# ArisKonidaris/OMLDM

Hardware: AMD Instinct MI355X
Metric: training examples/sec (whole node) + p50 predict latency, linear SVM 1/2/4/8 GPU (higher is better)
Workload: dtype fp32

## Files before the change

### csrc/kernels/linear_scan3.hip

```cpp
#include "common.h"
#include "hash_dev.h"
#include "seq_common.h"

namespace omldm {

typedef float f32x4 __attribute__((ext_vector_type(4)));

namespace s3 {
constexpr int CH = 64;
#ifndef OMLDM_S3_NH
#define OMLDM_S3_NH 11
#endif
constexpr int NH = OMLDM_S3_NH;
constexpr int NT = 64 * (NH + 1);
constexpr int WPE = (NH + 1 + 3) / 4;
constexpr int NHA = NH;
constexpr int GS = CH + 4;
constexpr int MAXF = 32;
constexpr int NF = (MAXF + NHA - 1) / NHA;
constexpr int KNMAX = 32;
constexpr int NJ = (KNMAX + NHA - 1) / NHA;
constexpr int MAT = CH * CH;
constexpr int RMAX = 8192;
constexpr int WS = 8;
constexpr int DS = KNMAX;
constexpr uint32_t F_TG = 1u;
constexpr uint32_t F_INIT = 2u;
constexpr uint32_t F_SCAT = 4u;
constexpr uint32_t F_SIGN = 8u;
constexpr uint32_t F_PRES = 16u;
constexpr uint32_t F_TAB = F_TG | F_INIT | F_SCAT;
constexpr int LID_SHIFT = 10;
}

template <int KN>
__host__ __device__ constexpr int s3_prep_floats() {
  return 2 * s3::MAT + s3::CH + KN * s3::CH + 3 * s3::CH;
}
template <int KN>
__host__ __device__ constexpr int s3_prep_y() {
  return 2 * s3::MAT + s3::CH + KN * s3::CH;
}
template <int KN>
__host__ __device__ constexpr int s3_prep_sg() {
  return s3_prep_y<KN>() + s3::CH;
}
template <int KN>
__host__ __device__ constexpr int s3_prep_hh() {
  return s3_prep_y<KN>() + 2 * s3::CH;
}
__device__ __forceinline__ float s3_shrink(int shr, float r, float tbase, int i, float y) {
  if (shr == 0 || y != y) return 1.f;
  if (shr == 2) {
    const float T = tbase + (float)i;
    return (T - 1.f) / T;
  }
  return r;
}

__device__ __forceinline__ void spoke_rows(int s, int R, int B, int& t0, int& t1) {
  const long long a = (long long)s * R;
  t0 = a > B ? B : (int)a;
  t1 = (a + R) > B ? B : (int)(a + R);
}

__global__ __launch_bounds__(256) void s3_slots_kernel(const void* __restrict__ src, int B,
                                                       int dc, int dn, uint32_t span, int hashed,
                                                       int cbase, int* __restrict__ slotsT) {
  __shared__ int tile[256][s3::MAXF + 1];
  const int r0 = blockIdx.x * 256, tid = threadIdx.x;
  const int nr = min(256, B - r0);
  for (int i = tid; i < nr * dc; i += 256) {
    const int r = i / dc, f = i - r * dc;
    int slot;
    if (hashed == 2) {
      const uint32_t v = reinterpret_cast<const uint16_t*>(src)[(size_t)r0 * dc + i];
      slot = v == 0xFFFFu ? -1
                          : (int)(((uint32_t)cbase + (uint32_t)f * span + (v & 0x7FFFu)) |
                                  ((v & 0x8000u) << 16));
    } else {
      const uint32_t v = reinterpret_cast<const uint32_t*>(src)[(size_t)r0 * dc + i];
      slot = hashed ? (int)v : hash_token_dev(v, f, dn, span);
    }
    tile[r][f] = slot;
  }
  __syncthreads();
  if (tid < nr)
    for (int f = 0; f < dc; ++f) slotsT[(size_t)f * B + r0 + tid] = tile[tid][f];
}

namespace s3 {
constexpr int FT = 1024;
constexpr int HCAP = 12288;
constexpr int RPT = RMAX / FT;
}

__global__ __launch_bounds__(s3::FT) void s3_flags_kernel(const int* __restrict__ slotsT, int B,
                                                          int R, uint32_t* __restrict__ meta,
                                                          int* __restrict__ lidcount, int enc,
                                                          int* __restrict__ l2s, long long gs) {
  __shared__ int hkey[s3::HCAP];
  __shared__ uint32_t hfirst[s3::HCAP];
  __shared__ uint32_t hlast[s3::HCAP];
  __shared__ int s_cnt, s_base;
// ... 621 lines not shown
  const int i = bid - base;
  s3_combine_spoke(slotsT, dc, B, R, cb, sm, i % cb.S_act, i / cb.S_act, (nblk - base) / cb.S_act);
}

__device__ void s3_dense_body(const float* __restrict__ ws, const float* __restrict__ wsd,
                              const float* __restrict__ sig, int S_act, int dn, int dim, int bias,
                              float inv_p, float* __restrict__ dacc, double* __restrict__ cum);

__device__ __forceinline__ void s3_scan_arrive(const S3Comb& cb, const float* __restrict__ ws,
                                               const float* __restrict__ wsd, int dn, int dim,
                                               const SeqParams& p, S3Smem& sm) {
  if (cb.arrive == nullptr) return;
  int& s_last = sm.last;
  asm volatile("s_waitcnt vmcnt(0)" ::: "memory");
  __syncthreads();
  if (threadIdx.x == 0) {
    __builtin_amdgcn_fence(__ATOMIC_RELEASE, "agent");
    asm volatile("s_waitcnt vmcnt(0)" ::: "memory");
    s3_gu64* a = (s3_gu64*)cb.arrive;
    unsigned long long old = __hip_atomic_load(a, __ATOMIC_RELAXED, __HIP_MEMORY_SCOPE_AGENT);
    unsigned long long nw;
    do {
      nw = (uint32_t)(old >> 32) == cb.epoch ? old + 1
                                             : (((unsigned long long)cb.epoch << 32) | 1ull);
    } while (!__hip_atomic_compare_exchange_weak(a, &old, nw, __ATOMIC_RELAXED,
                                                 __ATOMIC_RELAXED, __HIP_MEMORY_SCOPE_AGENT));
    s_last = (int)(uint32_t)nw == cb.S_act;
    if (s_last) {
      __builtin_amdgcn_fence(__ATOMIC_ACQUIRE, "agent");
      asm volatile("s_waitcnt vmcnt(0)" ::: "memory");
    }
  }
  __syncthreads();
  if (s_last)
    s3_dense_body(ws, wsd, cb.sig, cb.S_act, dn, dim, p.bias, p.inv_p, cb.dacc, cb.cum);
}

template <bool RARE>
__device__ __forceinline__ void s3_inscan_flush(const S3Comb& cb, const float* tab,
                                                float* ag, int cap,
                                                const float* __restrict__ w, int s) {
  __syncthreads();
  const int n = cb.lidcount[s];
  const float sc = cb.inv_p * (cb.sig ? cb.sig[s] : 1.f);
  const int* l2 = cb.l2s + (size_t)s * cb.gs;
  constexpr int FB = 8;
  for (int i0 = threadIdx.x; i0 < n; i0 += FB * s3::NT) {
    int slot[FB];
    float d[FB];
#pragma unroll
    for (int u = 0; u < FB; ++u) {
      const int i = i0 + u * s3::NT;
      slot[u] = l2[i < n ? i : 0];
    }
#pragma unroll
    for (int u = 0; u < FB; ++u) {
      const int i = i0 + u * s3::NT;
      d[u] = i < min(n, cap) ? tab[i] : 0.f;
    }
    if (n > cap) {
#pragma unroll
      for (int u = 0; u < FB; ++u) {
        const int i = i0 + u * s3::NT;
        if (i >= cap && i < n)
          d[u] = __hip_atomic_load(&ag[i - cap], __ATOMIC_RELAXED, __HIP_MEMORY_SCOPE_AGENT);
      }
    }
    if constexpr (!RARE) {
#pragma unroll
      for (int u = 0; u < FB; ++u) {
        const int i = i0 + u * s3::NT;
        const int sl = i < n ? slot[u] : 0;
        d[u] -= i < n ? (cb.wbf ? s3_w16(w, sl) : w[sl]) : 0.f;
      }
    }
#pragma unroll
    for (int u = 0; u < FB; ++u) {
      const int i = i0 + u * s3::NT;
      if (i < n && d[u] != 0.f) atomicAdd(&cb.dacc[slot[u]], sc * d[u]);
    }
  }
}

template <int RULE, int KN, bool RARE>
__device__ __forceinline__ void s3_scan_body(
    int bid, int nblk, S3Smem& sm, float* tab,
    const int* __restrict__ slotsT, const uint32_t* __restrict__ meta, int dc, int dn,
    const void* __restrict__ yv, int B, int R, const float* __restrict__ prep, int nchs,
    const float* __restrict__ w, int dim, float* __restrict__ aglob, int cap, long long gstride,
    const S3Comb& cb, float* __restrict__ ws, float* __restrict__ wsd, const SeqParams& p,
    unsigned long long* __restrict__ rgran) {
  constexpr int PF = s3_prep_floats<KN>();
  if (bid >= cb.S_act) {
    if (RARE && bid < 2 * cb.S_act) {
      s3_rare(slotsT, dc, B, R, w, cb, rgran, sm, bid - cb.S_act);
      if (cb.inscan == 2) s3_fold_pres(meta, dc, B, R, cb, bid - cb.S_act);
      return;
    }
    s3_combine(slotsT, dc, B, R, cb, sm, (RARE ? 2 : 1) * cb.S_act, bid, nblk);
    return;
  }
  const int tid = threadIdx.x;
  const int wave = __builtin_amdgcn_readfirstlane(tid >> 6), lane = tid & 63;
  const int s = bid;
  int t0, t1;
  spoke_rows(s, R, B, t0, t1);
  if (t0 >= t1) {
    if (tid < s3::WS) ws[(size_t)s * s3::WS + tid] = 0.f;
    if (tid < s3::DS) wsd[(size_t)s * s3::DS + tid] = 0.f;
    s3_scan_arrive(cb, ws, wsd, dn, dim, p, sm);
    return;
  }
  const int nch = (t1 - t0 + s3::CH - 1) / s3::CH;
  const float* P0 = prep + (size_t)s * nchs * PF;
  auto chunk_prep = [&](int k) { return P0 + (size_t)k * PF; };
  float* ag = aglob + (size_t)s * gstride;

  unsigned long long* stamps = g_s3_stamps;
  unsigned long long st_acc[12] = {};
  unsigned long long st_t = stamps ? clock64() : 0;
  auto stamp = [&](int k) {
    if (stamps) {
      const unsigned long long now = clock64();
      st_acc[k] += now - st_t;
      st_t = now;
    }
  };

  if (wave == 0) {
    __builtin_amdgcn_s_setprio(3);
    float loss = 0.f, nex = 0.f, mist = 0.f, sqe = 0.f;
    float f1 = 0.f;
    float ynx = chunk_prep(0)[s3_prep_y<KN>() + lane];
    float anx = chunk_prep(0)[2 * s3::MAT + lane];
    const bool shr = p.shr != 0;
    float snx = shr ? chunk_prep(0)[s3_prep_sg<KN>() + lane] : 1.f;
    float hnx = shr ? chunk_prep(0)[s3_prep_hh<KN>() + lane] : 1.f;
    for (int k = -1; k <= nch; ++k) {
      if (k >= 0 && k < nch) {
        const int b = k & 1;
        const int row = t0 + k * s3::CH + lane;
        const bool valid = row < t1 && ynx == ynx;
        const float y = valid ? ynx : 0.f;
        const float a = valid ? anx : 0.f;
        const float sg = valid ? snx : 1.f, hh = valid ? hnx : 1.f;
        if (k + 1 < nch) {
          ynx = chunk_prep(k + 1)[s3_prep_y<KN>() + lane];
          anx = chunk_prep(k + 1)[2 * s3::MAT + lane];
          if (shr) {
            snx = chunk_prep(k + 1)[s3_prep_sg<KN>() + lane];
            hnx = chunk_prep(k + 1)[s3_prep_hh<KN>() + lane];
          }
        }
        float m0 = 0.f;
#pragma unroll
        for (int q = 0; q < s3::NHA; ++q) m0 += sm.part[b][q][lane];
        S3Cand<RULE> cf;
        float u, bc = 0.f;
        const float inv = -a;
        if constexpr (RULE == kSeqHinge) {
          bc = y * inv * hh;
          cf.lo = y < 0.f ? -p.cclip * hh : 0.f;
          cf.hi = y < 0.f ? 0.f : (y > 0.f ? p.cclip * hh : 0.f);
          u = fmaf(a * (sg * hh), m0, bc) + f1;
        } else if constexpr (RULE == kSeqEps) {
          bc = (y - p.eps) * inv * hh;
          cf.d = 2.f * p.eps * inv * hh;
          cf.lo = valid ? -p.cclip * hh : 0.f;
          cf.hi = valid ? p.cclip * hh : 0.f;
          u = fmaf(a * (sg * hh), m0, bc) + f1;
        } else if constexpr (RULE == kSeqPegasos) {
          const float T = p.tbase + (float)(row - t0);
          cf.lo = valid ? 1.f / sg : 0.f;
          cf.hi = valid ? y * hh / (p.lam * T) : 0.f;
          u = fmaf(a, m0, 0.f) + f1;
        } else {
          cf.lo = y * sg;
          cf.hi = p.lr * y * hh;
          u = m0 + f1;
        }
        const float* grow = &sm.G[b][lane][0];
        const float* xrow = &sm.X1[b ^ 1][lane][0];
        float gg[s3::CH], xx[s3::CH];
#pragma unroll
        for (int t4 = 0; t4 < s3::CH; t4 += 4) {
          const float4 g4 = *reinterpret_cast<const float4*>(grow + t4);
          const float4 x4 = *reinterpret_cast<const float4*>(xrow + t4);
          gg[t4] = g4.x, gg[t4 + 1] = g4.y, gg[t4 + 2] = g4.z, gg[t4 + 3] = g4.w;
          xx[t4] = x4.x, xx[t4 + 1] = x4.y, xx[t4 + 2] = x4.z, xx[t4 + 3] = x4.w;
        }
        stamp(8);
        float n1 = 0.f;
        auto chain = [&](auto step) {
#pragma unroll
          for (int t = 0; t < s3::CH; ++t) {
            const float ct = readlane_f(step(u), t);
            u = fmaf(ct, gg[t], u);
            n1 = fmaf(ct, xx[t], n1);
            asm volatile("" : "+v"(u), "+v"(n1));
          }
        };
        if constexpr (RULE == kSeqLogistic) {
          if (!shr) {
            const float lo2 = y * 1.44269504088896341f;
            chain([&](float v) {
              return __builtin_amdgcn_rcpf(1.f + __builtin_amdgcn_exp2f(lo2 * v));
            });
          } else {
            chain([&](float v) { return cf(v, p, y); });
          }
        } else {
          chain([&](float v) { return cf(v, p, y); });
        }
        stamp(9);
        const float c = cf(u, p, y);
        sm.cb[b][lane] = c;
        if (row < t1 && cb.inscan != 1)
          __hip_atomic_store((s3_gu64*)(cb.gran + row),
                             ((unsigned long long)cb.epoch << 32) | __float_as_uint(c),
                             __ATOMIC_RELAXED, __HIP_MEMORY_SCOPE_AGENT);
        if (valid) {
          float m;
          if constexpr (RULE == kSeqLogistic) m = sg * u;
          else if constexpr (RULE == kSeqPegasos) m = sg * y * u;
          else m = inv > 0.f ? (bc - u) * __builtin_amdgcn_rcpf(inv * hh) : 0.f;
          seq_stats<RULE>(m, y, p, loss, mist, sqe);
          nex += 1.f;
        }
        f1 = n1;
      }
      stamp(0);
      __syncthreads();
      stamp(1);
    }
    if (stamps && lane == 0)
      for (int q = 0; q < 12; ++q)
        if (q < 2 || q >= 8) atomicAdd(&stamps[(size_t)s * 16 + q], st_acc[q]);
    loss = wave_sum(loss);
    nex = wave_sum(nex);
    mist = wave_sum(mist);
    sqe = wave_sum(sqe);
    if (lane == 0) {
      float* wr = ws + (size_t)s * s3::WS;
      wr[0] = loss;
      wr[1] = nex;
      wr[2] = mist;
      wr[3] = sqe;
      wr[4] = 1.f;
      wr[5] = 0.f;
      wr[6] = 0.f;
      wr[7] = 0.f;
    }
    if (cb.inscan) s3_inscan_flush<RARE>(cb, tab, ag, cap, w, s);
    s3_scan_arrive(cb, ws, wsd, dn, dim, p, sm);
    return;
  }

  const int q = wave - 1, r = lane;
  const int swave = g_s3_stamp_wave;
  const int kd = dn + (p.bias ? 1 : 0);
  const int hl = q * 64 + lane;
  const bool inscan = cb.inscan != 0, inscan1 = cb.inscan == 1;
  const uint32_t tmask = inscan ? s3::F_TAB : s3::F_SCAT;
  const float isc = inscan1 ? cb.inv_p * (cb.sig ? cb.sig[s] : 1.f) : 0.f;
  float wn[s3::NJ], w0[s3::NJ];
#pragma unroll
  for (int i = 0; i < s3::NJ; ++i) {
    const int j = q + s3::NHA * i;
    const int jw = j < dn ? j : dim - 1;
    const float wj = cb.wbf ? s3_w16(w, jw) : w[jw];
    w0[i] = (j < KN && (j < dn || (p.bias && j == dn))) ? wj : 0.f;
    wn[i] = w0[i];
  }
  constexpr int NV4 = (2 * s3::MAT / 4 + 64 * s3::NHA - 1) / (64 * s3::NHA);
  struct Set {
    int cs[s3::NF];
    uint32_t cm[s3::NF];
    float g[s3::NF];
    f32x4 v[NV4];
    float xs[s3::NJ], xc[s3::NJ];
    unsigned long long rg;
  };
  uint32_t p1[s3::NF], p2[s3::NF];
  const unsigned long long want = (unsigned long long)cb.epoch;
  bool dead = false;
  auto load_rare = [&](int ch) -> unsigned long long {
    const int row = t0 + ch * s3::CH + r;
    const bool ok = RARE && q == 0 && ch >= 0 && ch < nch && row < t1;
    return ok ? __hip_atomic_load((s3_gu64*)(rgran + row), __ATOMIC_RELAXED,
                                  __HIP_MEMORY_SCOPE_AGENT)
              : (want << 32);
  };
  auto load_words = [&](int ch, Set& S) {
    if constexpr (RARE) {
      S.rg = load_rare(ch);
#pragma unroll
      for (int i = 0; i < s3::NF; ++i) {
        const int f = q + s3::NHA * i;
        const int row = t0 + ch * s3::CH + r;
        const bool ok = ch >= 0 && ch < nch && f < dc && row < t1;
        const uint32_t mm = meta[ok ? (size_t)f * B + row : 0];
        S.cm[i] = ok ? mm : 0u;
        S.cs[i] = ok && (mm & (s3::F_TG | s3::F_INIT)) ? 0 : -1;
      }
      return;
    }
#pragma unroll
    for (int i = 0; i < s3::NF; ++i) {
      const int f = q + s3::NHA * i;
      const int row = t0 + ch * s3::CH + r;
      const bool ok = ch >= 0 && ch < nch && f < dc && row < t1;
      const size_t at = ok ? (size_t)f * B + row : 0;
      const int sl = slotsT[at];
      const uint32_t mm = meta[at];
      S.cs[i] = ok ? sl : -1;
      S.cm[i] = ok ? mm : 0u;
    }
  };
  auto issue_gathers = [&](Set& S) {
    if constexpr (RARE) return;
    if (cb.wbf) {
#pragma unroll
      for (int i = 0; i < s3::NF; ++i) {
        const bool glob = !RARE && S.cs[i] != -1 && !(S.cm[i] & s3::F_TG);
        S.g[i] = s3_w16(w, glob ? (S.cs[i] & 0x7fffffff) : 0);
      }
      return;
    }
#pragma unroll
    for (int i = 0; i < s3::NF; ++i) {
      const bool glob = !RARE && S.cs[i] != -1 && !(S.cm[i] & s3::F_TG);
      S.g[i] = w[glob ? (S.cs[i] & 0x7fffffff) : 0];
    }
  };
  auto issue_staging = [&](int ch, Set& S) {
#pragma unroll
    for (int u = 0; u < NV4; ++u) {
      const int i = min(hl + 64 * s3::NHA * u, 2 * s3::MAT / 4 - 1);
      const int mtx = i >> 10, e = i & 1023;
      const int kc = max(0, min(ch + mtx, nch - 1));
      S.v[u] = reinterpret_cast<const f32x4*>(chunk_prep(kc) + mtx * s3::MAT)[e];
    }
  };
  constexpr int NJK = (KN + s3::NHA - 1) / s3::NHA;
  auto load_dense = [&](int ch, float* xd) {
#pragma unroll
    for (int i = 0; i < NJK; ++i) {
      const int j = q + s3::NHA * i;
      const bool ok = j < KN && ch >= 0 && ch < nch;
      const int jc = j < KN ? j : 0, cc = max(0, min(ch, nch - 1));
      const float v = chunk_prep(cc)[2 * s3::MAT + s3::CH + jc * s3::CH + r];
      xd[i] = ok ? v : 0.f;
    }
  };
  auto body = [&](auto spill_tag, int k, Set& CUR, Set& NXT) {
    constexpr bool SPILL = decltype(spill_tag)::value;
    const int cn = k + 1, ks = k - 1;
    if (wave == swave) stamp(7);
    load_words(cn + 1, NXT);
    issue_staging(cn + 1, NXT);
    load_dense(ks + 1, NXT.xs);
    load_dense(cn + 1, NXT.xc);
    if (wave == swave) stamp(3);
    if (ks >= 0) {
      const float cv = sm.cb[ks & 1][r];
#pragma unroll
      for (int i = 0; i < s3::NF; ++i) {
        const uint32_t m = p2[i];
        const bool sc = (m & tmask) != 0u && cv != 0.f;
        const bool dr = inscan1 && (m & s3::F_PRES) != 0u && cv != 0.f;
        if (__builtin_amdgcn_ballot_w64(sc || dr) == 0ull) continue;
        const int lid = (int)(m >> s3::LID_SHIFT);
        const float val = (m & s3::F_SIGN) ? -cv : cv;
        if (dr) atomicAdd(&cb.dacc[lid], val * isc);
        if (sc) {
          if constexpr (SPILL) {
            if (lid < cap) atomicAdd(&tab[lid], val);
            else atomicAdd(&ag[lid - cap], val);
          } else {
            atomicAdd(&tab[lid], val);
          }
        }
      }
#pragma unroll
      for (int i = 0; i < NJK; ++i) {
        const int j = q + s3::NHA * i;
        if (j < kd) wn[i] += wave_sum(cv * CUR.xs[i]);
      }
    }
    if (wave == swave) stamp(6);
    if (cn < nch) {
      float base = 0.f;
#pragma unroll
      for (int i = 0; i < NJK; ++i) base = fmaf(CUR.xc[i], wn[i], base);
      if constexpr (RARE) {
        if (q == 0) {
          for (unsigned spins = 0;
               __builtin_amdgcn_ballot_w64((CUR.rg >> 32) != want) != 0ull;) {
            if (dead || ++spins > s3::SPIN_MAX) {
              if (!dead && r == 0) atomicExch(&g_s3_comb_err, 2);
              dead = true;
              break;
            }
            __builtin_amdgcn_s_sleep(1);
            CUR.rg = load_rare(cn);
          }
          base += (CUR.rg >> 32) == want ? __uint_as_float((uint32_t)CUR.rg) : 0.f;
        }
      }
      if constexpr (!SPILL) {
        float tv[s3::NF];
#pragma unroll
        for (int i = 0; i < s3::NF; ++i) {
          const uint32_t m = CUR.cm[i];
          const bool tg = CUR.cs[i] != -1 && (m & s3::F_TG);
          tv[i] = 0.f;
          if (tg) tv[i] = tab[(int)(m >> s3::LID_SHIFT)];
        }
#pragma unroll
        for (int i = 0; i < s3::NF; ++i) {
          const uint32_t m = CUR.cm[i];
          const bool here = CUR.cs[i] != -1;
          const bool tg = here && (m & s3::F_TG), init = here && !tg && (m & s3::F_INIT);
          const float val = tg ? tv[i] : (RARE ? 0.f : CUR.g[i]);
          if (init) tab[(int)(m >> s3::LID_SHIFT)] = val;
          if (here && (!RARE || tg)) base += (m & s3::F_SIGN) ? -val : val;
        }
      }
#pragma unroll
      for (int i = 0; SPILL && i < s3::NF; ++i) {
        const uint32_t m = CUR.cm[i];
        const bool here = CUR.cs[i] != -1;
        const int lid = (int)(m >> s3::LID_SHIFT);
        const bool tg = here && (m & s3::F_TG), init = here && !tg && (m & s3::F_INIT);
        float val = RARE ? 0.f : CUR.g[i];
        if (!SPILL || __builtin_amdgcn_ballot_w64((tg || init) && lid >= cap) == 0ull) {
          if (tg) val = tab[lid];
          if (init) tab[lid] = val;
        } else if constexpr (SPILL) {
          if (tg) val = lid < cap ? tab[lid] : __hip_atomic_load(&ag[lid - cap], __ATOMIC_RELAXED,
                                                                 __HIP_MEMORY_SCOPE_WORKGROUP);
          if (init) {
            if (lid < cap) tab[lid] = val;
            else __hip_atomic_store(&ag[lid - cap], val, __ATOMIC_RELAXED,
                                    __HIP_MEMORY_SCOPE_WORKGROUP);
          }
          asm volatile("s_waitcnt vmcnt(0)" ::: "memory");
        }
        if (here && (!RARE || tg)) base += (m & s3::F_SIGN) ? -val : val;
      }
      sm.part[cn & 1][q][r] = base;
    }
    if (wave == swave) stamp(4);
#pragma unroll
    for (int u = 0; u < NV4; ++u) {
      const int i = hl + 64 * s3::NHA * u;
      const int mtx = i >> 10, e = i & 1023;
      if (i < 2 * s3::MAT / 4 && cn + mtx < nch) {
        const int row = e >> 4, col = (e & 15) * 4;
        float* dst = mtx == 0 ? &sm.G[cn & 1][row][col] : &sm.X1[(cn + 1) & 1][row][col];
        *reinterpret_cast<f32x4*>(dst) = CUR.v[u];
      }
    }
    issue_gathers(NXT);
#pragma unroll
    for (int i = 0; i < s3::NF; ++i) {
      p2[i] = p1[i];
      p1[i] = CUR.cm[i];
    }
    if (wave == swave) stamp(5);
    __syncthreads();
  };

  Set A, Bs;
#pragma unroll
  for (int i = 0; i < s3::NF; ++i) p1[i] = p2[i] = 0u;
  load_words(0, A);
  issue_staging(0, A);
  load_dense(-2, A.xs);
  load_dense(0, A.xc);
  issue_gathers(A);
  if (cb.lidcount[s] <= cap) {
    for (int k = -1; k <= nch; k += 2) {
      body(S3Tag<false>{}, k, A, Bs);
      if (k + 1 <= nch) body(S3Tag<false>{}, k + 1, Bs, A);
    }
  } else {
    for (int k = -1; k <= nch; k += 2) {
      body(S3Tag<true>{}, k, A, Bs);
      if (k + 1 <= nch) body(S3Tag<true>{}, k + 1, Bs, A);
    }
  }
  if (stamps && lane == 0 && wave == swave)
    for (int k = 2; k < 8; ++k) atomicAdd(&stamps[(size_t)s * 16 + k], st_acc[k]);
#pragma unroll
  for (int i = 0; i < s3::NJ; ++i) {
    const int j = q + s3::NHA * i;
    if (lane == 0 && j < KN) wsd[(size_t)s * s3::DS + j] = wn[i] - w0[i];
  }
  if (q == 0 && lane >= KN && lane < s3::DS) wsd[(size_t)s * s3::DS + lane] = 0.f;
  if (cb.inscan) s3_inscan_flush<RARE>(cb, tab, ag, cap, w, s);
  s3_scan_arrive(cb, ws, wsd, dn, dim, p, sm);
}

constexpr int kS3MaxPipes = 16;
struct S3Pipe {
  const float* w;
  float* aglob;
  float* ws;
  float* wsd;
  unsigned long long* rgran;
  S3Comb cb;
  SeqParams p;
};
struct S3Pipes {
  int M;
  int ncomb;
  const unsigned long long* wflag;
  unsigned long long wepoch;
  S3Pipe pipe[kS3MaxPipes];
};

__global__ void s3_signal_kernel(unsigned long long* flag, unsigned long long epoch) {
  if (threadIdx.x == 0)
    __hip_atomic_store(flag, epoch, __ATOMIC_RELEASE, __HIP_MEMORY_SCOPE_AGENT);
}

__device__ __forceinline__ void s3_wait_prep(const unsigned long long* flag,
                                             unsigned long long epoch) {
  if (flag == nullptr) return;
  if (threadIdx.x == 0) {
    for (unsigned spins = 0;
         __hip_atomic_load(flag, __ATOMIC_RELAXED, __HIP_MEMORY_SCOPE_AGENT) < epoch;) {
      if (++spins > s3::SPIN_MAX) {
        atomicExch(&g_s3_comb_err, 3);
        break;
      }
      __builtin_amdgcn_s_sleep(2);
    }
    __builtin_amdgcn_fence(__ATOMIC_ACQUIRE, "agent");
  }
  __syncthreads();
}

template <int RULE, int KN, bool RARE>
__global__ __launch_bounds__(s3::NT, s3::WPE) __attribute__((amdgpu_waves_per_eu(s3::WPE, s3::WPE))) void s3_scan_kernel(
    const int* __restrict__ slotsT, const uint32_t* __restrict__ meta, int dc, int dn,
    const void* __restrict__ yv, int B, int R, const float* __restrict__ prep, int nchs,
    int dim, int cap, long long gstride, int S_act, S3Pipes pp) {
  __shared__ S3Smem sm;
  extern __shared__ float tab[];
  const int nblk = s3_nper(S_act, RARE, pp.ncomb);
  const int pi = (int)blockIdx.x / nblk, local = (int)blockIdx.x % nblk;
  s3_wait_prep(pp.wflag, pp.wepoch);
  int bid;
  if (RARE && local < S_act) bid = S_act + local;
  else if (RARE && local < 2 * S_act) bid = local - S_act;
  else bid = local;
  const S3Pipe& P = pp.pipe[pi];
  s3_scan_body<RULE, KN, RARE>(bid, nblk, sm, tab, slotsT, meta, dc, dn, yv, B, R, prep, nchs,
                               P.w, dim, P.aglob, cap, gstride, P.cb, P.ws, P.wsd, P.p, P.rgran);
}

__device__ void s3_dense_body(const float* __restrict__ ws,
                              const float* __restrict__ wsd, const float* __restrict__ sig,
                              int S_act, int dn, int dim, int bias, float inv_p,
                              float* __restrict__ dacc,
                              double* __restrict__ cum) {
  const int tid = threadIdx.x;
  const bool bad = __hip_atomic_load(&g_s3_comb_err, __ATOMIC_RELAXED, __HIP_MEMORY_SCOPE_AGENT) != 0;
  for (int i = tid; i < dn; i += 256) {
    float v = 0.f;
    for (int s = 0; s < S_act; ++s) v += wsd[(size_t)s * s3::DS + i] * (sig ? sig[s] : 1.f);
    dacc[i] = v * inv_p;
  }
  if (tid == 0) {
    float v = 0.f, a = 0.f;
    if (bias)
      for (int s = 0; s < S_act; ++s) v += wsd[(size_t)s * s3::DS + dn] * (sig ? sig[s] : 1.f);
    for (int s = 0; s < S_act; ++s) a += sig ? sig[s] : 1.f;
    dacc[dim - 1] = v * inv_p;
    dacc[dim] = a * inv_p;
    dacc[dim + 1] = bad ? -1e30f : (float)S_act * inv_p;
  }
  if (cum && !bad && tid < 6 && tid != 4) {
    double t = 0.0;
    for (int s = 0; s < S_act; ++s) t += (double)ws[(size_t)s * s3::WS + tid];
    cum[tid] += t;
  }
}

namespace s3 {
constexpr int SB = 4096;
constexpr int SH = 4096;
constexpr int SPROBE = 8;
}

__global__ __launch_bounds__(256) void s3_tail_kernel(const float* __restrict__ ws,
                                                      const float* __restrict__ wsd,
                                                      const float* __restrict__ sig, int S_act,
                                                      int dn, int dim, int bias, float inv_p,
                                                      float* __restrict__ dacc,
                                                      double* __restrict__ cum) {
  s3_dense_body(ws, wsd, sig, S_act, dn, dim, bias, inv_p, dacc, cum);
}

__global__ __launch_bounds__(256) void s3_scatter_kernel(const int* __restrict__ slotsT,
                                                         const unsigned long long* __restrict__ gran, int B,
                                                         int n_rows, float inv_p,
                                                         float* __restrict__ dacc, int dc,
                                                         const float* __restrict__ ws,
                                                         const float* __restrict__ wsd, int S_act,
                                                         int dn, int dim, int bias,
                                                         double* __restrict__ cum, int R,
                                                         const float* __restrict__ sig) {
  if ((int)blockIdx.y == dc) {
    if (blockIdx.x == 0) s3_dense_body(ws, wsd, sig, S_act, dn, dim, bias, inv_p, dacc, cum);
    return;
  }
  __shared__ int hk[s3::SH];
  __shared__ float hv[s3::SH];
  const int f = blockIdx.y, tid = threadIdx.x;
  const int r0 = blockIdx.x * s3::SB, r1 = min(n_rows, r0 + s3::SB);
  for (int i = tid; i < s3::SH; i += 256) {
    hk[i] = -1;
    hv[i] = 0.f;
  }
  __syncthreads();
  const int* col = slotsT + (size_t)f * B;
  for (int row = r0 + tid; row < r1; row += 256) {
    const int v = col[row];
    if (v == -1) continue;
    const float c = __uint_as_float((uint32_t)gran[row]);
    if (c == 0.f) continue;
    const int key = v & 0x7fffffff;
    const float sc = sig ? inv_p * sig[row / R] : inv_p;
    const float val = v < 0 ? -c * sc : c * sc;
    uint32_t at = ((uint32_t)key * 0x9E3779B1u) >> (32 - 12);
    bool done = false;
    for (int probe = 0; probe < s3::SPROBE; ++probe) {
      const int prev = atomicCAS(&hk[at], -1, key);
      if (prev == -1 || prev == key) {
        atomicAdd(&hv[at], val);
// ... 484 lines not shown
  }
#pragma unroll
  for (int i = 0; i < s3::NJ; ++i) {
    const int j = q + s3::NHA * i;
    if (lane == 0 && j < s3::DS)
#pragma unroll
      for (int c = 0; c < K; ++c)
        A.wsd[((size_t)s * K + c) * s3::DS + j] =
            (i < NJK0 && j < KN) ? wn[c][i < NJK0 ? i : 0] - w0_at(i, c) : 0.f;
  }
  if (hdbg && lane == 0) {
    atomicAdd(&hdbg[s * 8 + 3], h_sc);
    atomicAdd(&hdbg[s * 8 + 4], h_mg);
    atomicAdd(&hdbg[s * 8 + 5], h_st);
    atomicAdd(&hdbg[s * 8 + 6], h_wt);
    if (q == 0) atomicAdd(&hdbg[s * 8 + 7], (unsigned long long)(lidcount[s] > capid));
  }
}

__global__ __launch_bounds__(256) void s3mc_scatter_kernel(
    const int* __restrict__ slotsT, const float* __restrict__ tau, const int* __restrict__ rr,
    const void* __restrict__ yv, int y8, int nclass, int B, int n_rows, float* __restrict__ dacc,
    int dim, int dc, int dn, int bias, int K, int KN, const float* __restrict__ ws,
    const float* __restrict__ wsd, int S_act, float* __restrict__ stats) {
  if ((int)blockIdx.y == dc) {
    if (blockIdx.x != 0) return;
    const int tid = threadIdx.x;
    for (int i = tid; i < K * KN; i += 256) {
      const int c = i / KN, j = i - c * KN;
      if (j >= dn + (bias ? 1 : 0) || c >= nclass) continue;
      float v = 0.f;
      for (int s = 0; s < S_act; ++s) v += wsd[((size_t)s * K + c) * s3::DS + j];
      const int key = j < dn ? j : dim - 1;
      dacc[(size_t)c * dim + key] += v;
    }
    if (tid < 3) {
      float t = 0.f;
      for (int s = 0; s < S_act; ++s) t += ws[(size_t)s * s3::WS + tid];
      stats[tid] += t;
    }
    if (tid == 3) stats[3] += (float)S_act;
    return;
  }
  __shared__ int hk[s3::SH];
  __shared__ float hv[s3::SH];
  const int f = blockIdx.y, tid = threadIdx.x;
  const int r0 = blockIdx.x * s3::SB, r1 = min(n_rows, r0 + s3::SB);
  for (int i = tid; i < s3::SH; i += 256) {
    hk[i] = -1;
    hv[i] = 0.f;
  }
  __syncthreads();
  const int* col = slotsT + (size_t)f * B;
  auto add = [&](int key, float val) {
    uint32_t at = ((uint32_t)key * 0x9E3779B1u) >> (32 - 12);
    for (int probe = 0; probe < s3::SPROBE; ++probe) {
      const int prev = atomicCAS(&hk[at], -1, key);
      if (prev == -1 || prev == key) {
        atomicAdd(&hv[at], val);
        return;
      }
      at = (at + 1) & (s3::SH - 1);
    }
    atomicAdd(&dacc[key], val);
  };
  for (int row = r0 + tid; row < r1; row += 256) {
    const int v = col[row];
    const float t = tau[row];
    if (v == -1 || t == 0.f) continue;
    const int slot = v & 0x7fffffff;
    const float val = v < 0 ? -t : t;
    const float yf = load_y(yv, row, y8);
    const int yc = (yf == yf && yf >= 0.f && yf < (float)nclass) ? (int)yf : -1;
    if (yc >= 0) add(yc * dim + slot, val);
    if (rr[row] >= 0) add(rr[row] * dim + slot, -val);
  }
  __syncthreads();
  for (int i = tid; i < s3::SH; i += 256) {
    const int key = hk[i];
    if (key != -1) atomicAdd(&dacc[key], hv[i]);
  }
}

template <int RULE, int KN, bool RARE>
static int s3_launch_scan_t(const int* slotsT, const uint32_t* meta, int dc, int dn, const void* y,
                            int B, int R, int S_act, const float* prep, int nchs, int dim, int cap,
                            long long gstride, const S3Pipes& pp, hipStream_t st) {
  static bool attr_set = false;
  if (!attr_set) {
    hipFuncSetAttribute(reinterpret_cast<const void*>(&s3_scan_kernel<RULE, KN, RARE>),
                        hipFuncAttributeMaxDynamicSharedMemorySize,
                        160 * 1024 - (int)sizeof(S3Smem));
    attr_set = true;
  }
  const int nblk = pp.M * s3_nper(S_act, RARE, pp.ncomb);
  hipLaunchKernelGGL((s3_scan_kernel<RULE, KN, RARE>), dim3(nblk), dim3(s3::NT),
                     (size_t)(cap + 64) * sizeof(float), st, slotsT, meta, dc, dn, y, B, R, prep,
                     nchs, dim, cap, gstride, S_act, pp);
  return (int)hipGetLastError();
}

template <int KN>
static int s3_launch_scan(int rule, bool rare, const int* slotsT, const uint32_t* meta, int dc,
                          int dn, const void* y, int B, int R, int S_act, const float* prep,
                          int nchs, int dim, int cap, long long gstride, const S3Pipes& pp,
                          hipStream_t st) {
#define OMLDM_S3L(RL, RA) \
  return s3_launch_scan_t<RL, KN, RA>(slotsT, meta, dc, dn, y, B, R, S_act, prep, nchs, dim, cap, \
                                      gstride, pp, st)
  if (rare) {
    if (rule == kSeqHinge) OMLDM_S3L(kSeqHinge, true);
    if (rule == kSeqEps) OMLDM_S3L(kSeqEps, true);
    if (rule == kSeqPegasos) OMLDM_S3L(kSeqPegasos, true);
    OMLDM_S3L(kSeqLogistic, true);
  }
  if (rule == kSeqHinge) OMLDM_S3L(kSeqHinge, false);
  if (rule == kSeqEps) OMLDM_S3L(kSeqEps, false);
  if (rule == kSeqPegasos) OMLDM_S3L(kSeqPegasos, false);
  OMLDM_S3L(kSeqLogistic, false);
#undef OMLDM_S3L
}

}

using namespace omldm;

namespace {
int s3_sact(int B, int R, int S) {
  const long long sact = ((long long)B + R - 1) / R;
  return sact < S ? (int)sact : S;
}
int s3_kn(int dn, int bias) { return dn + (bias ? 1 : 0) <= 16 ? 16 : 32; }
constexpr size_t kFlagsLds = (size_t)s3::HCAP * 12;
}

static int g_s3_cap_override = -1;

static int g_s3_mode = 4;
static int g_s3_inscan = 1;
OMLDM_API void omldm_scan3_set_inscan(int v) { g_s3_inscan = v; }
OMLDM_API void omldm_scan3_set_mode(int m) { g_s3_mode = m == 3 ? 3 : 4; }
OMLDM_API int omldm_scan3_get_mode() { return g_s3_mode; }

OMLDM_API int omldm_scan3_lds_cap() {
  const int hw = (int)((160 * 1024 - sizeof(S3Smem)) / sizeof(float)) - 64;
  return g_s3_cap_override >= 0 && g_s3_cap_override < hw ? g_s3_cap_override : hw;
}

OMLDM_API void omldm_scan3_set_cap(int cap) { g_s3_cap_override = cap; }

static int g_s3_gram_valu = 0;
OMLDM_API void omldm_scan3_set_gram_valu(int v) { g_s3_gram_valu = v; }

static int g_s3_comb = 1;
OMLDM_API void omldm_scan3_set_comb(int v) { g_s3_comb = v < 0 ? 0 : (v > 3 ? 3 : v); }
OMLDM_API int omldm_scan3_get_comb() { return g_s3_comb; }

OMLDM_API int omldm_scan3_comb_err() {
  int v = 0, z = 0;
  if (hipMemcpyFromSymbol(&v, HIP_SYMBOL(g_s3_comb_err), sizeof(v)) != hipSuccess) return -1;
  if (v) hipMemcpyToSymbol(HIP_SYMBOL(g_s3_comb_err), &z, sizeof(z));
  return v;
}

__global__ void s3_err_drain_kernel(int* out) {
  if (threadIdx.x == 0) {
    const int v = atomicExch(&g_s3_comb_err, 0);
    out[0] = v > out[0] ? v : out[0];
  }
}

OMLDM_API int omldm_scan3_comb_err_drain(int* out, void* stream) {
  hipLaunchKernelGGL(s3_err_drain_kernel, dim3(1), dim3(64), 0, (hipStream_t)stream, out);
  return (int)hipGetLastError();
}

OMLDM_API int omldm_scan3_fits(int dn, int dc, int R, int bias) {
  return dc > 0 && dc <= s3::MAXF && dn >= 0 && dn + (bias ? 1 : 0) <= s3::KNMAX && R > 0 &&
         R <= s3::RMAX;
}

OMLDM_API long long omldm_scan3_ws_words(int which, int B, int R, int S, int dn, int dc,
// ... 304 lines not shown
```

### omldm_amd/cli.py

```python
from __future__ import annotations

import json
import sys

from omldm_amd.utils.config import JobConfig, argparser


def main(argv=None) -> int:
    argv = list(sys.argv[1:] if argv is None else argv)
    if "-h" in argv or "--help" in argv:
        argparser().print_help()
        return 0
    cfg = JobConfig.from_args(argv)
    from omldm_amd.engine.job import Job
    from omldm_amd.parallel.comm import init_distributed

    comm, device = init_distributed(cfg.device)
    job = Job(cfg, comm, device).run()
    if comm.rank == 0:
        print(json.dumps({"job": cfg.jobName, "ticks": job.ticks, "counters": job.counters,
                          "terminated": job.terminated}), flush=True)
    return 0


if __name__ == "__main__":
    sys.exit(main())
```

### omldm_amd/parallel/comm.py

```python
from __future__ import annotations

import os
from dataclasses import dataclass, field

import torch
import torch.distributed as dist


_BYTE_WIRE = (torch.int16, torch.uint16, torch.bool) if hasattr(torch, "uint16") else \
    (torch.int16, torch.bool)


@dataclass
class CommStats:
    collectives: int = 0
    bytes: int = 0
    small_collectives: int = 0
    per_tag: dict = field(default_factory=dict)
    trace: list | None = None

    def add(self, tag: str, nbytes: int, small: bool = False, kind: str = "all_reduce"):
        if self.trace is not None:
            self.trace.append((kind, tag, int(nbytes)))
        self.collectives += 1
# ... 153 lines not shown
    def broadcast_(self, t: torch.Tensor, src: int = 0, tag: str = "bcast"):
        if self.world > 1:
            self.stats.add(tag, t.numel() * t.element_size(), kind="broadcast")
            dist.broadcast(t, src=src, group=self.group)

    def broadcast_object(self, obj, src: int = 0):
        if self.world == 1:
            return obj
        box = [obj if self.rank == src else None]
        dist.broadcast_object_list(box, src=src, group=self.group)
        return box[0]

    def all_gather_object(self, obj) -> list:
        if self.world == 1:
            return [obj]
        out = [None] * self.world
        dist.all_gather_object(out, obj, group=self.group)
        return out

    def gather_tensor(self, t: torch.Tensor, dst: int = 0) -> list[torch.Tensor] | None:
        if self.world == 1:
            return [t]
        n = torch.tensor([t.shape[0]], dtype=torch.int64)
        ns_t = [torch.zeros_like(n) for _ in range(self.world)] if self.rank == dst else None
        dist.gather(n, ns_t, dst=dst, group=self.ctrl_group)
        wire_dtype = t.dtype
        src = t.contiguous()
        if wire_dtype in _BYTE_WIRE:
            src = src.view(torch.uint8)
        row_shape = tuple(src.shape[1:])
        if self.rank != dst:
            if t.shape[0]:
                self.stats.add("gather", src.numel() * src.element_size(), kind="p2p_send")
                dist.send(src, dst=dst, group=self.group)
            return None
        ns = [int(x[0]) for x in ns_t]
        outs, works = [], []
        for r, k in enumerate(ns):
            if r == dst:
                outs.append(src)
                continue
            buf = torch.empty((k,) + row_shape, dtype=src.dtype, device=src.device)
            outs.append(buf)
            if k:
                works.append(dist.irecv(buf, src=r, group=self.group))
        for w in works:
            w.wait()
        if wire_dtype in _BYTE_WIRE:
            outs = [o.view(wire_dtype) for o in outs]
        return outs

    def barrier(self):
        if self.world > 1:
            dist.barrier(group=self.group)


def init_distributed(device_type: str = "auto", timeout_s: float = 600.0) -> tuple[Comm, torch.device]:
    import datetime

    world = int(os.environ.get("WORLD_SIZE", "1"))
    rank = int(os.environ.get("RANK", "0"))
    local_rank = int(os.environ.get("LOCAL_RANK", "0"))
    use_gpu = torch.cuda.is_available() if device_type == "auto" else device_type != "cpu"
    backend = os.environ.get("OMLDM_DIST_BACKEND") or ("nccl" if use_gpu else "gloo")
    ndev = torch.cuda.device_count() if use_gpu else 0
    device = torch.device("cuda", local_rank % max(1, ndev)) if use_gpu else torch.device("cpu")
    placement = {}
    if use_gpu:
        torch.cuda.set_device(device)
        from omldm_amd.utils.topology import bind_to_device

        placement = bind_to_device(device)
    if world > 1 and not dist.is_initialized():
        os.environ.setdefault("MASTER_ADDR", "127.0.0.1")
        os.environ.setdefault("MASTER_PORT", "29533")
        kw = {}
        if use_gpu and backend == "nccl":
            kw["device_id"] = device
        dist.init_process_group(backend, rank=rank, world_size=world,
                                timeout=datetime.timedelta(seconds=timeout_s), **kw)
    comm = Comm()
    comm.placement = placement
    return comm, device
```

Before: 343.8 million.

## Dedicate last wave to LDS-direct staging and rare-granule waits in scan kernel

The last wave of each scan block becomes a producer. It streams the G and X1 matrices straight into LDS with global_load_lds and handles the rare-granule spin-wait. The remaining helper waves split the fields across one fewer wave and no longer hold staging registers, which should free VGPRs and take the staging traffic off the compute path. A template parameter NFQ picks a smaller per-wave field count when dc is small, and rare helpers now sleep briefly each iteration. The risks are fewer compute waves per field and added coupling to the barrier protocol; a distributed shutdown call is also added.

Result: no change. 344.5 million (median of 3 runs) (+0.2%).

```diff
diff --git a/csrc/kernels/linear_scan3.hip b/csrc/kernels/linear_scan3.hip
--- a/csrc/kernels/linear_scan3.hip
+++ b/csrc/kernels/linear_scan3.hip
@@ -1,6 +1,7 @@
 #include "common.h"
 #include "hash_dev.h"
 #include "seq_common.h"
+#include "s3_stage_map.h"
 
 namespace omldm {
 
@@ -20,6 +21,11 @@
 constexpr int NF = (MAXF + NHA - 1) / NHA;
 constexpr int KNMAX = 32;
 constexpr int NJ = (KNMAX + NHA - 1) / NHA;
+constexpr int NFH = NH - 1;
+constexpr int NFB = (MAXF + NFH - 1) / NFH;
+constexpr int NJB = (KNMAX + NFH - 1) / NFH;
+constexpr int HEAD_SLEEP = 8;
+static_assert(NFH >= 1 && NFH < NHA, "the staging wave's partial row follows the field helpers'");
 constexpr int MAT = CH * CH;
 constexpr int RMAX = 8192;
 constexpr int WS = 8;
@@ -807,7 +813,7 @@
   }
 }
 
-template <int RULE, int KN, bool RARE>
+template <int RULE, int KN, bool RARE, int NFQ>
 __device__ __forceinline__ void s3_scan_body(
     int bid, int nblk, S3Smem& sm, float* tab,
     const int* __restrict__ slotsT, const uint32_t* __restrict__ meta, int dc, int dn,
@@ -842,7 +848,7 @@
   float* ag = aglob + (size_t)s * gstride;
 
   unsigned long long* stamps = g_s3_stamps;
-  unsigned long long st_acc[12] = {};
+  unsigned long long st_acc[14] = {};
   unsigned long long st_t = stamps ? clock64() : 0;
   auto stamp = [&](int k) {
     if (stamps) {
@@ -981,47 +987,94 @@
     return;
   }
 
+  if (wave == s3::NH) {
+    typedef __attribute__((address_space(1))) const char s3_gsrc;
+    typedef __attribute__((address_space(3))) char s3_ldst;
+    static_assert(sizeof(sm.G[0]) == s3::STG_N * s3::STG_LROW &&
+                      sizeof(sm.X1[0]) == s3::STG_N * s3::STG_LROW && s3::MAT == s3::STG_N * s3::STG_N,
+                  "s3_stage_map.h maps the scan's G / X1 image");
+    uint32_t soff[s3::STG_PIECES];
+#pragma unroll
+    for (int u = 0; u < s3::STG_PIECES; ++u) soff[u] = s3::stage_src(u, lane);
+    auto stage = [&](const float* src, float* dst) {
+#pragma unroll
+      for (int u = 0; u < s3::STG_PIECES; ++u)
+        __builtin_amdgcn_global_load_lds((s3_gsrc*)src + soff[u],
+                                         (s3_ldst*)dst + u * s3::STG_PIECE, 16, 0, 0);
+    };
+    const unsigned long long want = (unsigned long long)cb.epoch;
+    bool dead = false;
+    auto load_rare = [&](int ch) -> unsigned long long {
+      const int row = t0 + ch * s3::CH + lane;
+      return row < t1 ? __hip_atomic_load((s3_gu64*)(rgran + row), __ATOMIC_RELAXED,
+                                          __HIP_MEMORY_SCOPE_AGENT)
+                      : (want << 32);
+    };
+    for (int k = -1; k <= nch; ++k) {
+      const int cn = k + 1;
+      stamp(13);
+      if (cn < nch) stage(chunk_prep(cn), &sm.G[cn & 1][0][0]);
+      if (cn + 1 < nch) stage(chunk_prep(cn + 1) + s3::MAT, &sm.X1[(cn + 1) & 1][0][0]);
+      stamp(10);
+      unsigned long long rg = want << 32;
+      if constexpr (RARE) {
+        if (cn < nch) rg = load_rare(cn);
+      }
+      asm volatile("s_waitcnt vmcnt(0)" ::: "memory");
+      stamp(11);
+      if (cn < nch) {
+        float rm = 0.f;
+        if constexpr (RARE) {
+          for (unsigned spins = 0; __builtin_amdgcn_ballot_w64((rg >> 32) != want) != 0ull;) {
+            if (dead || ++spins > s3::SPIN_MAX) {
+              if (!dead && lane == 0) atomicExch(&g_s3_comb_err, 2);
+              dead = true;
+              break;
+            }
+            __builtin_amdgcn_s_sleep(1);
+            rg = load_rare(cn);
+          }
+          rm = (rg >> 32) == want ? __uint_as_float((uint32_t)rg) : 0.f;
+        }
+        sm.part[cn & 1][s3::NFH][lane] = rm;
+      }
+      stamp(12);
+      __syncthreads();
+    }
+    if (stamps && lane == 0)
+      for (int k = 10; k < 14; ++k) atomicAdd(&stamps[(size_t)s * 16 + k], st_acc[k]);
+    if (cb.inscan) s3_inscan_flush<RARE>(cb, tab, ag, cap, w, s);
+    s3_scan_arrive(cb, ws, wsd, dn, dim, p, sm);
+    return;
+  }
+
   const int q = wave - 1, r = lane;
   const int swave = g_s3_stamp_wave;
   const int kd = dn + (p.bias ? 1 : 0);
-  const int hl = q * 64 + lane;
   const bool inscan = cb.inscan != 0, inscan1 = cb.inscan == 1;
   const uint32_t tmask = inscan ? s3::F_TAB : s3::F_SCAT;
   const float isc = inscan1 ? cb.inv_p * (cb.sig ? cb.sig[s] : 1.f) : 0.f;
-  float wn[s3::NJ], w0[s3::NJ];
-#pragma unroll
-  for (int i = 0; i < s3::NJ; ++i) {
-    const int j = q + s3::NHA * i;
+  float wn[s3::NJB], w0[s3::NJB];
+#pragma unroll
+  for (int i = 0; i < s3::NJB; ++i) {
+    const int j = q + s3::NFH * i;
     const int jw = j < dn ? j : dim - 1;
     const float wj = cb.wbf ? s3_w16(w, jw) : w[jw];
     w0[i] = (j < KN && (j < dn || (p.bias && j == dn))) ? wj : 0.f;
     wn[i] = w0[i];
   }
-  constexpr int NV4 = (2 * s3::MAT / 4 + 64 * s3::NHA - 1) / (64 * s3::NHA);
   struct Set {
-    int cs[s3::NF];
-    uint32_t cm[s3::NF];
-    float g[s3::NF];
-    f32x4 v[NV4];
-    float xs[s3::NJ], xc[s3::NJ];
-    unsigned long long rg;
+    int cs[NFQ];
+    uint32_t cm[NFQ];
+    float g[NFQ];
+    float xs[s3::NJB], xc[s3::NJB];
   };
-  uint32_t p1[s3::NF], p2[s3::NF];
-  const unsigned long long want = (unsigned long long)cb.epoch;
-  bool dead = false;
-  auto load_rare = [&](int ch) -> unsigned long long {
-    const int row = t0 + ch * s3::CH + r;
-    const bool ok = RARE && q == 0 && ch >= 0 && ch < nch && row < t1;
-    return ok ? __hip_atomic_load((s3_gu64*)(rgran + row), __ATOMIC_RELAXED,
-                                  __HIP_MEMORY_SCOPE_AGENT)
-              : (want << 32);
-  };
+  uint32_t p1[NFQ], p2[NFQ];
   auto load_words = [&](int ch, Set& S) {
     if constexpr (RARE) {
-      S.rg = load_rare(ch);
-#pragma unroll
-      for (int i = 0; i < s3::NF; ++i) {
-        const int f = q + s3::NHA * i;
+#pragma unroll
+      for (int i = 0; i < NFQ; ++i) {
+        const int f = q + s3::NFH * i;
         const int row = t0 + ch * s3::CH + r;
         const bool ok = ch >= 0 && ch < nch && f < dc && row < t1;
         const uint32_t mm = meta[ok ? (size_t)f * B + row : 0];
@@ -1031,8 +1084,8 @@
       return;
     }
 #pragma unroll
-    for (int i = 0; i < s3::NF; ++i) {
-      const int f = q + s3::NHA * i;
+    for (int i = 0; i < NFQ; ++i) {
+      const int f = q + s3::NFH * i;
       const int row = t0 + ch * s3::CH + r;
       const bool ok = ch >= 0 && ch < nch && f < dc && row < t1;
       const size_t at = ok ? (size_t)f * B + row : 0;
@@ -1046,32 +1099,23 @@
     if constexpr (RARE) return;
     if (cb.wbf) {
 #pragma unroll
-      for (int i = 0; i < s3::NF; ++i) {
+      for (int i = 0; i < NFQ; ++i) {
         const bool glob = !RARE && S.cs[i] != -1 && !(S.cm[i] & s3::F_TG);
         S.g[i] = s3_w16(w, glob ? (S.cs[i] & 0x7fffffff) : 0);
       }
       return;
     }
 #pragma unroll
-    for (int i = 0; i < s3::NF; ++i) {
+    for (int i = 0; i < NFQ; ++i) {
       const bool glob = !RARE && S.cs[i] != -1 && !(S.cm[i] & s3::F_TG);
       S.g[i] = w[glob ? (S.cs[i] & 0x7fffffff) : 0];
     }
   };
-  auto issue_staging = [&](int ch, Set& S) {
-#pragma unroll
-    for (int u = 0; u < NV4; ++u) {
-      const int i = min(hl + 64 * s3::NHA * u, 2 * s3::MAT / 4 - 1);
-      const int mtx = i >> 10, e = i & 1023;
-      const int kc = max(0, min(ch + mtx, nch - 1));
-      S.v[u] = reinterpret_cast<const f32x4*>(chunk_prep(kc) + mtx * s3::MAT)[e];
-    }
-  };
-  constexpr int NJK = (KN + s3::NHA - 1) / s3::NHA;
+  constexpr int NJK = (KN + s3::NFH - 1) / s3::NFH;
   auto load_dense = [&](int ch, float* xd) {
 #pragma unroll
     for (int i = 0; i < NJK; ++i) {
-      const int j = q + s3::NHA * i;
+      const int j = q + s3::NFH * i;
       const bool ok = j < KN && ch >= 0 && ch < nch;
       const int jc = j < KN ? j : 0, cc = max(0, min(ch, nch - 1));
       const float v = chunk_prep(cc)[2 * s3::MAT + s3::CH + jc * s3::CH + r];
@@ -1083,14 +1127,14 @@
     const int cn = k + 1, ks = k - 1;
     if (wave == swave) stamp(7);
     load_words(cn + 1, NXT);
-    issue_staging(cn + 1, NXT);
     load_dense(ks + 1, NXT.xs);
     load_dense(cn + 1, NXT.xc);
     if (wave == swave) stamp(3);
+    if constexpr (RARE) __builtin_amdgcn_s_sleep(s3::HEAD_SLEEP);
     if (ks >= 0) {
       const float cv = sm.cb[ks & 1][r];
 #pragma unroll
-      for (int i = 0; i < s3::NF; ++i) {
+      for (int i = 0; i < NFQ; ++i) {
         const uint32_t m = p2[i];
         const bool sc = (m & tmask) != 0u && cv != 0.f;
         const bool dr = inscan1 && (m & s3::F_PRES) != 0u && cv != 0.f;
@@ -1109,7 +1153,7 @@
       }
 #pragma unroll
       for (int i = 0; i < NJK; ++i) {
-        const int j = q + s3::NHA * i;
+        const int j = q + s3::NFH * i;
         if (j < kd) wn[i] += wave_sum(cv * CUR.xs[i]);
       }
     }
@@ -1118,32 +1162,17 @@
       float base = 0.f;
 #pragma unroll
       for (int i = 0; i < NJK; ++i) base = fmaf(CUR.xc[i], wn[i], base);
-      if constexpr (RARE) {
-        if (q == 0) {
-          for (unsigned spins = 0;
-               __builtin_amdgcn_ballot_w64((CUR.rg >> 32) != want) != 0ull;) {
-            if (dead || ++spins > s3::SPIN_MAX) {
-              if (!dead && r == 0) atomicExch(&g_s3_comb_err, 2);
-              dead = true;
-              break;
-            }
-            __builtin_amdgcn_s_sleep(1);
-            CUR.rg = load_rare(cn);
-          }
-          base += (CUR.rg >> 32) == want ? __uint_as_float((uint32_t)CUR.rg) : 0.f;
-        }
-      }
       if constexpr (!SPILL) {
-        float tv[s3::NF];
-#pragma unroll
-        for (int i = 0; i < s3::NF; ++i) {
+        float tv[NFQ];
+#pragma unroll
+        for (int i = 0; i < NFQ; ++i) {
           const uint32_t m = CUR.cm[i];
           const bool tg = CUR.cs[i] != -1 && (m & s3::F_TG);
           tv[i] = 0.f;
           if (tg) tv[i] = tab[(int)(m >> s3::LID_SHIFT)];
         }
 #pragma unroll
-        for (int i = 0; i < s3::NF; ++i) {
+        for (int i = 0; i < NFQ; ++i) {
           const uint32_t m = CUR.cm[i];
           const bool here = CUR.cs[i] != -1;
           const bool tg = here && (m & s3::F_TG), init = here && !tg && (m & s3::F_INIT);
@@ -1153,7 +1182,7 @@
         }
       }
 #pragma unroll
-      for (int i = 0; SPILL && i < s3::NF; ++i) {
+      for (int i = 0; SPILL && i < NFQ; ++i) {
         const uint32_t m = CUR.cm[i];
         const bool here = CUR.cs[i] != -1;
         const int lid = (int)(m >> s3::LID_SHIFT);
@@ -1177,19 +1206,9 @@
       sm.part[cn & 1][q][r] = base;
     }
     if (wave == swave) stamp(4);
-#pragma unroll
-    for (int u = 0; u < NV4; ++u) {
-      const int i = hl + 64 * s3::NHA * u;
-      const int mtx = i >> 10, e = i & 1023;
-      if (i < 2 * s3::MAT / 4 && cn + mtx < nch) {
-        const int row = e >> 4, col = (e & 15) * 4;
-        float* dst = mtx == 0 ? &sm.G[cn & 1][row][col] : &sm.X1[(cn + 1) & 1][row][col];
-        *reinterpret_cast<f32x4*>(dst) = CUR.v[u];
-      }
-    }
     issue_gathers(NXT);
 #pragma unroll
-    for (int i = 0; i < s3::NF; ++i) {
+    for (int i = 0; i < NFQ; ++i) {
       p2[i] = p1[i];
       p1[i] = CUR.cm[i];
     }
@@ -1199,9 +1218,8 @@
 
   Set A, Bs;
 #pragma unroll
-  for (int i = 0; i < s3::NF; ++i) p1[i] = p2[i] = 0u;
+  for (int i = 0; i < NFQ; ++i) p1[i] = p2[i] = 0u;
   load_words(0, A);
-  issue_staging(0, A);
   load_dense(-2, A.xs);
   load_dense(0, A.xc);
   issue_gathers(A);
@@ -1219,8 +1237,8 @@
   if (stamps && lane == 0 && wave == swave)
     for (int k = 2; k < 8; ++k) atomicAdd(&stamps[(size_t)s * 16 + k], st_acc[k]);
 #pragma unroll
-  for (int i = 0; i < s3::NJ; ++i) {
-    const int j = q + s3::NHA * i;
+  for (int i = 0; i < s3::NJB; ++i) {
+    const int j = q + s3::NFH * i;
     if (lane == 0 && j < KN) wsd[(size_t)s * s3::DS + j] = wn[i] - w0[i];
   }
   if (q == 0 && lane >= KN && lane < s3::DS) wsd[(size_t)s * s3::DS + lane] = 0.f;
@@ -1268,7 +1286,7 @@
   __syncthreads();
 }
 
-template <int RULE, int KN, bool RARE>
+template <int RULE, int KN, bool RARE, int NFQ>
 __global__ __launch_bounds__(s3::NT, s3::WPE) __attribute__((amdgpu_waves_per_eu(s3::WPE, s3::WPE))) void s3_scan_kernel(
     const int* __restrict__ slotsT, const uint32_t* __restrict__ meta, int dc, int dn,
     const void* __restrict__ yv, int B, int R, const float* __restrict__ prep, int nchs,
@@ -1283,7 +1301,7 @@
   else if (RARE && local < 2 * S_act) bid = local - S_act;
   else bid = local;
   const S3Pipe& P = pp.pipe[pi];
-  s3_scan_body<RULE, KN, RARE>(bid, nblk, sm, tab, slotsT, meta, dc, dn, yv, B, R, prep, nchs,
+  s3_scan_body<RULE, KN, RARE, NFQ>(bid, nblk, sm, tab, slotsT, meta, dc, dn, yv, B, R, prep, nchs,
                                P.w, dim, P.aglob, cap, gstride, P.cb, P.ws, P.wsd, P.p, P.rgran);
 }
 
@@ -1934,22 +1952,33 @@
   }
 }
 
+template <int RULE, int KN, bool RARE, int NFQ>
+static int s3_launch_scan_q(const int* slotsT, const uint32_t* meta, int dc, int dn, const void* y,
+                            int B, int R, int S_act, const float* prep, int nchs, int dim, int cap,
+                            long long gstride, const S3Pipes& pp, hipStream_t st) {
+  static bool attr_set = false;
+  if (!attr_set) {
+    hipFuncSetAttribute(reinterpret_cast<const void*>(&s3_scan_kernel<RULE, KN, RARE, NFQ>),
+                        hipFuncAttributeMaxDynamicSharedMemorySize,
+                        160 * 1024 - (int)sizeof(S3Smem));
+    attr_set = true;
+  }
+  const int nblk = pp.M * s3_nper(S_act, RARE, pp.ncomb);
+  hipLaunchKernelGGL((s3_scan_kernel<RULE, KN, RARE, NFQ>), dim3(nblk), dim3(s3::NT),
+                     (size_t)(cap + 64) * sizeof(float), st, slotsT, meta, dc, dn, y, B, R, prep,
+                     nchs, dim, cap, gstride, S_act, pp);
+  return (int)hipGetLastError();
+}
+
 template <int RULE, int KN, bool RARE>
 static int s3_launch_scan_t(const int* slotsT, const uint32_t* meta, int dc, int dn, const void* y,
                             int B, int R, int S_act, const float* prep, int nchs, int dim, int cap,
                             long long gstride, const S3Pipes& pp, hipStream_t st) {
-  static bool attr_set = false;
-  if (!attr_set) {
-    hipFuncSetAttribute(reinterpret_cast<const void*>(&s3_scan_kernel<RULE, KN, RARE>),
-                        hipFuncAttributeMaxDynamicSharedMemorySize,
-                        160 * 1024 - (int)sizeof(S3Smem));
-    attr_set = true;
-  }
-  const int nblk = pp.M * s3_nper(S_act, RARE, pp.ncomb);
-  hipLaunchKernelGGL((s3_scan_kernel<RULE, KN, RARE>), dim3(nblk), dim3(s3::NT),
-                     (size_t)(cap + 64) * sizeof(float), st, slotsT, meta, dc, dn, y, B, R, prep,
-                     nchs, dim, cap, gstride, S_act, pp);
-  return (int)hipGetLastError();
+  if (dc <= (s3::NFB - 1) * s3::NFH)
+    return s3_launch_scan_q<RULE, KN, RARE, s3::NFB - 1>(slotsT, meta, dc, dn, y, B, R, S_act, prep,
+                                                         nchs, dim, cap, gstride, pp, st);
+  return s3_launch_scan_q<RULE, KN, RARE, s3::NFB>(slotsT, meta, dc, dn, y, B, R, S_act, prep, nchs,
+                                                   dim, cap, gstride, pp, st);
 }
 
 template <int KN>
diff --git a/csrc/kernels/s3_stage_map.h b/csrc/kernels/s3_stage_map.h
--- /dev/null
+++ b/csrc/kernels/s3_stage_map.h
@@ -0,0 +1,48 @@
+#pragma once
+#include <cstdint>
+
+namespace omldm {
+namespace s3 {
+constexpr int STG_N = 64;
+constexpr int STG_SROW = STG_N * 4;
+constexpr int STG_LROW = (STG_N + 4) * 4;
+constexpr int STG_PIECE = 64 * 16;
+constexpr int STG_PIECES = STG_N * STG_LROW / STG_PIECE;
+static_assert(STG_PIECES * STG_PIECE == STG_N * STG_LROW, "the image is whole pieces");
+static_assert(STG_LROW % 16 == 0 && STG_SROW % 16 == 0, "a lane's 16 bytes stay in one row");
+
+constexpr uint32_t stage_src(int u, int lane) {
+  const int o = u * STG_PIECE + 16 * lane;
+  const int row = o / STG_LROW, col = o % STG_LROW;
+  return (uint32_t)(row * STG_SROW + (col < STG_SROW ? col : 0));
+}
+
+constexpr bool stage_map_image_ok() {
+  for (int row = 0; row < STG_N; ++row)
+    for (int c = 0; c < STG_N; ++c) {
+      const int o = row * STG_LROW + 4 * c;
+      const int u = o / STG_PIECE, lane = (o % STG_PIECE) / 16, e = (o % 16) / 4;
+      if (u >= STG_PIECES) return false;
+      if (stage_src(u, lane) + 4u * e != (uint32_t)(row * STG_N + c) * 4u) return false;
+    }
+  return true;
+}
+constexpr bool stage_map_cover_ok() {
+  int hits[STG_N * STG_N / 4] = {};
+  for (int u = 0; u < STG_PIECES; ++u)
+    for (int lane = 0; lane < 64; ++lane) {
+      const int o = u * STG_PIECE + 16 * lane;
+      const uint32_t src = stage_src(u, lane);
+      if (src % 16u != 0u || src + 16u > (uint32_t)(STG_N * STG_SROW)) return false;
+      if (o + 16 > STG_N * STG_LROW) return false;
+      if (o % STG_LROW < STG_SROW) ++hits[src / 16u];
+    }
+  for (int i = 0; i < STG_N * STG_N / 4; ++i)
+    if (hits[i] != 1) return false;
+  return true;
+}
+static_assert(STG_PIECES == 17, "17 LDS-direct loads per matrix");
+static_assert(stage_map_image_ok(), "LDS float [row][c] receives matrix element [row][c]");
+static_assert(stage_map_cover_ok(), "sources tile the matrix once and stay inside it");
+}
+}
diff --git a/omldm_amd/cli.py b/omldm_amd/cli.py
--- a/omldm_amd/cli.py
+++ b/omldm_amd/cli.py
@@ -13,13 +13,14 @@
         return 0
     cfg = JobConfig.from_args(argv)
     from omldm_amd.engine.job import Job
-    from omldm_amd.parallel.comm import init_distributed
+    from omldm_amd.parallel.comm import init_distributed, shutdown_distributed
 
     comm, device = init_distributed(cfg.device)
     job = Job(cfg, comm, device).run()
     if comm.rank == 0:
         print(json.dumps({"job": cfg.jobName, "ticks": job.ticks, "counters": job.counters,
                           "terminated": job.terminated}), flush=True)
+    shutdown_distributed()
     return 0
 
 
diff --git a/omldm_amd/parallel/comm.py b/omldm_amd/parallel/comm.py
--- a/omldm_amd/parallel/comm.py
+++ b/omldm_amd/parallel/comm.py
@@ -259,3 +259,8 @@
     comm = Comm()
     comm.placement = placement
     return comm, device
+
+
+def shutdown_distributed() -> None:
+    if dist.is_available() and dist.is_initialized():
+        dist.destroy_process_group()
```
